# hkust-vgd/pointwise

Hardware: AMD Instinct MI355X
Metric: conv3p fwd+bwd Mpoints/s (higher is better)
Workload: dtype f32; 1 GPU; cfg2 ModelNet40-shaped: B=32 clouds/GPU x N=2048, pointcnn2_acsd conv3p stack 3->9 s1, 9->9 s2, 9->9 s3, 9->9 s4 (+SELU), forward+backward, a different batch every step, next batch's neighbour search enqueued on a side stream under the current backward; global_batch=32, points_per_cloud=2048, parallelism=dp1, backward_kernel_choice=hint from Conv3pStack.tune() at set-up: short lists

## Files before the change

pointwise_amd/csrc/conv3p_search_fused.hpp:

```cpp
#pragma once

#include "conv3p_device.hpp"

namespace conv3p {

constexpr int kFR = 16;
constexpr int kFK = 96;
constexpr int kFEntries = 116;
constexpr int kFHeader = 3 * kFEntries;
constexpr int kFTableU64 = kFHeader + 4;
constexpr int kFMaxExt = 8;
#ifndef CONV3P_DEV_FUSED_ABLATE
#define CONV3P_DEV_FUSED_ABLATE 0
#endif
constexpr int kFStream = 192;
constexpr int kFMaxE = 12;

__device__ __forceinline__ int floor_i32(float x)
{
    int r;
    asm("v_cvt_flr_i32_f32_e32 %0, %1" : "=v"(r) : "v"(x));
    return r;
}
__device__ __forceinline__ bool finite3(float x, float y, float z)
{
    return (x - x) + (y - y) + (z - z) == 0.0f;
}

__host__ __device__ constexpr int fused_window(int es) { return (kFR >> es) >= 1 ? (kFR >> es) + 1 : 2; }
static_assert(kFEntries >= kFK + fused_window(0) + 1 && kFEntries % 2 == 0, "window entries per axis");

template <typename T>
__global__ __launch_bounds__(256) void tile_tables_kernel(const PointRec<T> *__restrict__ pts, int ntiles, float inv16,
                                                          unsigned long long *__restrict__ tables,
                                                          const uint32_t *__restrict__ version,
                                                          uint32_t *__restrict__ tab_version,
                                                          uint32_t *__restrict__ tab_ticket,
                                                          uint32_t *__restrict__ tab_inv,
                                                          int force)
{
    __shared__ __attribute__((aligned(16))) unsigned long long tab[kWavesPerBlock][kFTableU64];
    const int wave = threadIdx.x >> 6, lane = threadIdx.x & 63;
    const int tile = blockIdx.x * kWavesPerBlock + wave;
    const int b = blockIdx.y;
    if (tile >= ntiles) return;
    if (!force && tab_version[b] == version[b] && tab_inv[b] == __builtin_bit_cast(uint32_t, inv16)) return;
    const size_t t = (size_t)b * ntiles + tile;
    const PointRec<T> r = pts[t * kTile + lane];
    const float v[3] = {(float)r.x, (float)r.y, (float)r.z};
    const bool valid = r.idx >= 0 && finite3(v[0], v[1], v[2]);
    float tmin[3], ext = 0.0f;
#pragma unroll
    for (int a = 0; a < 3; ++a) {
        tmin[a] = wave_min(valid ? v[a] : __builtin_huge_valf());
        const float tmax = wave_max(valid ? v[a] : -__builtin_huge_valf());
        ext = fmaxf(ext, (tmax - tmin[a]) * inv16);
    }
    const uint64_t allv = __ballot(valid);
    int e = 0;
    if (allv == 0) {
        tmin[0] = tmin[1] = tmin[2] = 0.0f;
    } else if (!(ext < 1.0e30f)) {
        e = kFMaxE + 1;
    } else {
        while (e <= kFMaxE && floor_i32(ext) >> e > kFK - 1) ++e;
    }
    const int es = e > 31 ? 31 : e;
    const int ws = fused_window(es);
    int beta[3];
#pragma unroll
    for (int a = 0; a < 3; ++a) {
        int b16 = floor_i32((v[a] - tmin[a]) * inv16) >> es;
        b16 = b16 < 0 ? 0 : (b16 > kFK - 1 ? kFK - 1 : b16);
        beta[a] = b16;
    }
    unsigned long long *mytab = tab[wave];
    {
        uint4 *z = reinterpret_cast<uint4 *>(mytab);
        for (int i = lane; i < kFTableU64 / 2; i += 64) z[i] = make_uint4(0, 0, 0, 0);
    }
    __builtin_amdgcn_wave_barrier();
    if (valid) {
        const unsigned long long bit = 1ull << lane;
        for (int i = 1; i <= ws; ++i) {
#pragma unroll
            for (int a = 0; a < 3; ++a) atomicOr(&mytab[a * kFEntries + beta[a] + i], bit);
        }
    }
    __builtin_amdgcn_wave_barrier();
    if (lane == 0) {
        mytab[kFHeader + 0] = (uint64_t)__builtin_bit_cast(uint32_t, tmin[0]) | ((uint64_t)__builtin_bit_cast(uint32_t, tmin[1]) << 32);
        mytab[kFHeader + 1] = (uint64_t)__builtin_bit_cast(uint32_t, tmin[2]) | ((uint64_t)(uint32_t)e << 32);
        mytab[kFHeader + 2] = allv;
        mytab[kFHeader + 3] = 0;
    }
    __builtin_amdgcn_wave_barrier();
    __builtin_amdgcn_s_waitcnt(0xc07f);
    const uint4 *src = reinterpret_cast<const uint4 *>(mytab);
    uint4 *dst = reinterpret_cast<uint4 *>(tables + t * kFTableU64);
    for (int i = lane; i < kFTableU64 / 2; i += 64) dst[i] = src[i];
    if (!force && lane == 0) {
        const uint32_t done = atomicAdd(&tab_ticket[b], 1u);
        if (done + 1u == (uint32_t)ntiles) {
            tab_inv[b] = __builtin_bit_cast(uint32_t, inv16);
            tab_version[b] = version[b];
            tab_ticket[b] = 0;
        }
    }
}

template <typename T> struct FusedJob {
    Stencil<T> st;
    CacheCtl cc;
    int32_t *count, *tcount;
    PairEntry *pairs;
    uint2 *segs, *qsegs;
    uint32_t *qbm, *qbm_hi;
    float clo[3][kFMaxExt];
};
constexpr int kFusedMaxJobs = 8;
template <typename T> struct FusedJobs {
    FusedJob<T> job[kFusedMaxJobs];
};

struct FusedLds {
    size_t tapmap, cnt, cen, bmk, nqw, misc, red, tab, masks, stream, total;
};
__host__ __device__ inline size_t f_a16(size_t x) { return (x + 15) & ~(size_t)15; }
__host__ __device__ inline FusedLds fused_lds(int ntap, int maxfull, int elem, int M)
{
    FusedLds L;
    size_t off = 0;
    L.tapmap = off; off += f_a16((size_t)3 * maxfull * 2);
    L.cnt = off; off += f_a16((size_t)ntap * kCntStride * 4);
    L.cen = off; off += (size_t)64 * 12 * elem;
    L.bmk = off; off += (ntap > 64 ? 256 : ntap > 32 ? 128 : 64) * 4;
    L.nqw = off; off += (size_t)kWavesPerBlock * 64 * 4;
    L.misc = off; off += 16;
    L.red = off; off += 6 * 8;
    off = f_a16(off);
    L.tab = off; off += (size_t)kWavesPerBlock * kFTableU64 * 8;
    L.masks = off; off += (size_t)kWavesPerBlock * M * 64 * 8;
    L.stream = off; off += (size_t)kWavesPerBlock * 2 * kFStream * 4;
    L.total = off;
    return L;
}

template <typename T>
__device__ __forceinline__ uint64_t tiles_meeting(const T *__restrict__ cloud_box, int ntiles, int base, const T *ulo, const T *uhi)
{
    const int t = base + (threadIdx.x & 63);
    bool ov = false;
    if (t < ntiles) {
        const T *bb = cloud_box + (size_t)t * 6;
        const T b0 = bb[0], b1 = bb[1], b2 = bb[2], b3 = bb[3], b4 = bb[4], b5 = bb[5];
        ov = !((b3 < ulo[0]) | (b0 > uhi[0]) | (b4 < ulo[1]) | (b1 > uhi[1]) | (b5 < ulo[2]) | (b2 > uhi[2]));
    }
    return __ballot(ov);
}

template <typename T>
__device__ __forceinline__ uint64_t fused_mask(const FusedJob<T> &job, const unsigned long long *tab, const float *gs, const float *fz,
                                               bool qvalid, int e)
{
    uint64_t H = ~0ull;
#pragma unroll
    for (int a = 0; a < 3; ++a) {
        uint64_t A = 0;
        const unsigned long long *ta = tab + a * kFEntries;
        for (int k = 0; k < job.st.ext[a]; ++k) {
            const float x = gs[a] + job.clo[a][k];
            int j = floor_i32(x) >> e, jh = floor_i32(x + fz[a]) >> e;
            j = j < 0 ? 0 : (j > kFEntries - 1 ? kFEntries - 1 : j);
            jh = jh < 0 ? 0 : (jh > kFEntries - 1 ? kFEntries - 1 : jh);
            A |= ta[j];
            if (__any(qvalid && jh != j)) A |= ta[jh];
        }
        H &= A;
    }
    return H;
}

template <typename T> struct TapFast {
    static constexpr bool enabled = false;
};
template <> struct TapFast<float> {
    static constexpr bool enabled = true;
};
__device__ __forceinline__ float min3_t(float a, float b, float c) { return fminf(fminf(a, b), c); }
__device__ __forceinline__ double min3_t(double a, double b, double c) { return fmin(fmin(a, b), c); }
__device__ __forceinline__ int clamp_tap(int t, int full)
{
    t = t > full - 1 ? full - 1 : t;
    return t < 0 ? 0 : t;
}

template <typename T> struct __attribute__((aligned(16))) CenRec {
    T lo[3], hi[3], p[3];
    T pad[3];
};

template <typename T>
__device__ __forceinline__ void fused_resolve(const Stencil<T> &st, T rvoxel, const int16_t *tapmap, uint32_t *cnt, uint32_t *bmk,
                                              const CenRec<T> *cen, uint32_t ql, const PointRec<T> &v, bool on, bool want_bwd,
                                              bool want_bm, uint32_t &fwd, uint32_t &bwd)
{
    const CenRec<T> c = cen[ql];
    const T d[3] = {v.x - c.lo[0], v.y - c.lo[1], v.z - c.lo[2]};
    const T dm = min3_t(d[0], d[1], d[2]);
    const T em = min3_t(c.hi[0] - v.x, c.hi[1] - v.y, c.hi[2] - v.z);
    const bool in = on && dm >= (T)0 && em >= (T)0;
    const T vv[3] = {v.x, v.y, v.z};
    fwd = kNoTap;
    bwd = kNoTap;
    bool exact = in;
    if (TapFast<T>::enabled) {
        int t[3];
        bool near = false;
#pragma unroll
        for (int a = 0; a < 3; ++a) {
            const float q = (float)d[a] * (float)rvoxel;
            const float mag = fmaxf(fabsf((float)c.p[a]), fabsf((float)vv[a]));
            near |= fabsf(q - __builtin_rintf(q)) <= __builtin_fmaf(mag, 5.0e-7f * (float)rvoxel, 1.0e-6f * (float)st.full[a]);
            t[a] = (int)q;
        }
        exact = in && near;
        if (in && !near) {
            const int tx = tapmap[clamp_tap(t[0], st.full[0])];
            const int ty = tapmap[st.maxfull + clamp_tap(t[1], st.full[1])];
            const int tz = tapmap[2 * st.maxfull + clamp_tap(t[2], st.full[2])];
            if ((tx | ty | tz) >= 0) {
                fwd = (uint32_t)((tz * st.ext[1] + ty) * st.ext[0] + tx);
                bwd = (uint32_t)st.ntap - 1u - fwd;
            }
        }
    }
    if (exact) {
        const int tx = tapmap[clamp_tap((int)(d[0] / st.voxel), st.full[0])];
        const int ty = tapmap[st.maxfull + clamp_tap((int)(d[1] / st.voxel), st.full[1])];
        const int tz = tapmap[2 * st.maxfull + clamp_tap((int)(d[2] / st.voxel), st.full[2])];
        if ((tx | ty | tz) >= 0) {
            fwd = (uint32_t)((tz * st.ext[1] + ty) * st.ext[0] + tx);
            if (want_bwd) {
                const T lx = (T)((double)v.x - st.half[0]), ly = (T)((double)v.y - st.half[1]), lz = (T)((double)v.z - st.half[2]);
                const int bx = tapmap[clamp_tap((int)((c.p[0] - lx) / st.voxel), st.full[0])];
                const int by = tapmap[st.maxfull + clamp_tap((int)((c.p[1] - ly) / st.voxel), st.full[1])];
                const int bz = tapmap[2 * st.maxfull + clamp_tap((int)((c.p[2] - lz) / st.voxel), st.full[2])];
                if ((bx | by | bz) >= 0) bwd = (uint32_t)((bz * st.ext[1] + by) * st.ext[0] + bx);
            }
        }
    }
    if (fwd != kNoTap) {
        atomicAdd(&cnt[fwd * kCntStride + ql], 1u);
        if (want_bm && bwd != kNoTap) atomicOr(&bmk[ql + ((bwd >> 5) << 6)], 1u << (bwd & 31u));
    }
}

typedef int int4_a4 __attribute__((ext_vector_type(4), aligned(4)));

constexpr uint32_t kFHitsOf32Neighbours = 40;
template <typename T> __device__ __forceinline__ bool fused_compacts(const Stencil<T> &st, uint32_t tile_hits)
{
    return !(CONV3P_DEV_FUSED_ABLATE & 16) && tile_hits > kFHitsOf32Neighbours * 64u;
}

template <typename T, bool EXT3>
__global__ __launch_bounds__(256) void search_fused_kernel(const PointRec<T> *__restrict__ pts, const T *__restrict__ boxes,
                                                           const unsigned long long *__restrict__ tables, int N, int ntiles,
                                                           int ngroups, BlockMap bm, FusedJobs<T> jobs, int M, float inv16)
{
    extern __shared__ __attribute__((aligned(16))) char smem[];
    const int wave = threadIdx.x >> 6, lane = threadIdx.x & 63;
    int b, qt;
    if (!block_to_cloud(bm, b, qt)) return;
    const FusedJob<T> &job = jobs.job[blockIdx.y];
    const bool have_pairs = job.pairs != nullptr;
    if (have_pairs && slot_valid(job.cc, b)) return;
    const Stencil<T> &st = job.st;

    const FusedLds L = fused_lds(st.ntap, st.maxfull, (int)sizeof(T), M);
    int16_t *tapmap = reinterpret_cast<int16_t *>(smem + L.tapmap);
    uint32_t *cnt = reinterpret_cast<uint32_t *>(smem + L.cnt);
    CenRec<T> *cen = reinterpret_cast<CenRec<T> *>(smem + L.cen);
    uint32_t *bmk = reinterpret_cast<uint32_t *>(smem + L.bmk);
    uint32_t *nqw = reinterpret_cast<uint32_t *>(smem + L.nqw);
    uint32_t *misc = reinterpret_cast<uint32_t *>(smem + L.misc);
    T *red = reinterpret_cast<T *>(smem + L.red);
    unsigned long long *tab = reinterpret_cast<unsigned long long *>(smem + L.tab) + (size_t)wave * kFTableU64;
    unsigned long long *masks = reinterpret_cast<unsigned long long *>(smem + L.masks) + (size_t)wave * M * 64;

    const PointRec<T> *cloud_pts = pts + (size_t)b * ntiles * kTile;
    const T *cloud_box = boxes + (size_t)b * ntiles * 6;
    const unsigned long long *cloud_tab = tables + (size_t)b * ntiles * kFTableU64;
    const PointRec<T> me = cloud_pts[(size_t)qt * kTile + lane];
    const float pf[3] = {(float)me.x, (float)me.y, (float)me.z};
    const bool qvalid = me.idx >= 0 && finite3(pf[0], pf[1], pf[2]);
    const bool want_bm = job.qbm != nullptr && (st.ntap <= 32 || (st.ntap <= 128 && job.qbm_hi != nullptr));

    build_tapmap(tapmap, st.full, st.step, st.maxfull);
    for (int e = threadIdx.x; e < st.ntap * kCntStride; e += blockDim.x) cnt[e] = 0;
    if (wave == 0) {
        CenRec<T> r;
        const T p[3] = {me.x, me.y, me.z};
#pragma unroll
        for (int a = 0; a < 3; ++a) {
            r.lo[a] = (T)((double)p[a] - st.half[a]);
            r.hi[a] = (T)((double)p[a] + st.half[a]);
            r.p[a] = p[a];
            r.pad[a] = (T)0;
        }
        cen[lane] = r;
        bmk[lane] = 0;
        if (st.ntap > 32) bmk[64 + lane] = 0;
        if (st.ntap > 64) bmk[128 + lane] = bmk[192 + lane] = 0;
    } else {
        const int a = wave - 1;
        const T pa = a == 0 ? me.x : (a == 1 ? me.y : me.z);
        const T mn = wave_min(qvalid ? pa : Limits<T>::inf()), mx = wave_max(qvalid ? pa : -Limits<T>::inf());
        if (lane == 0) {
            red[a] = mn;
            red[3 + a] = mx;
        }
    }
    const float q0[3] = {1.0e-3f + 4.0e-6f * (fabsf(pf[0]) * inv16), 1.0e-3f + 4.0e-6f * (fabsf(pf[1]) * inv16),
                         1.0e-3f + 4.0e-6f * (fabsf(pf[2]) * inv16)};
    __syncthreads();
    T ulo[3], uhi[3];
#pragma unroll
    for (int a = 0; a < 3; ++a) {
        ulo[a] = (T)((double)red[a] - st.half[a]);
        uhi[a] = (T)((double)red[3 + a] + st.half[a]);
    }
    const int S16[3] = {kFR * st.step[0], kFR * st.step[1], kFR * st.step[2]};

    auto for_my_tiles = [&](auto &&visit) {
        for (int base = 0; base < ntiles; base += 64) {
            uint64_t todo = tiles_meeting(cloud_box, ntiles, base, ulo, uhi) & (0x1111111111111111ull << wave);
            while (todo) {
                const int i = __builtin_ctzll(todo);
                todo &= todo - 1;
                visit(base + i, todo ? base + __builtin_ctzll(todo) : -1);
            }
        }
    };
    uint4 pf0 = make_uint4(0, 0, 0, 0), pf1 = pf0, pf2 = pf0;
    int pf_ct = -1;
    auto request = [&](int ct) {
        const uint4 *src = reinterpret_cast<const uint4 *>(cloud_tab + (size_t)ct * kFTableU64);
        pf0 = src[lane];
        pf1 = src[64 + lane];
        pf2 = src[128 + (lane < kFTableU64 / 2 - 128 ? lane : 0)];
        pf_ct = ct;
    };
    auto compute_mask = [&](int ct, int nxt) -> uint64_t {
        if (pf_ct != ct) request(ct);
        uint4 *dst = reinterpret_cast<uint4 *>(tab);
        __builtin_amdgcn_wave_barrier();
        dst[lane] = pf0;
        dst[64 + lane] = pf1;
        if (lane < kFTableU64 / 2 - 128) dst[128 + lane] = pf2;
        __builtin_amdgcn_wave_barrier();
        if (nxt >= 0) request(nxt);
        if (CONV3P_DEV_FUSED_ABLATE & 4) return 0ull;
        const uint64_t h0 = tab[kFHeader], h1 = tab[kFHeader + 1];
        const float tmin[3] = {__builtin_bit_cast(float, (uint32_t)h0), __builtin_bit_cast(float, (uint32_t)(h0 >> 32)),
                               __builtin_bit_cast(float, (uint32_t)h1)};
        const int e = (int)(uint32_t)(h1 >> 32);
        const int es = e > kFMaxE ? kFMaxE : e;
        const int ws = fused_window(es);
        float gs[3], fz[3], smax = 0.0f;
#pragma unroll
        for (int a = 0; a < 3; ++a) {
            const float g = (pf[a] - tmin[a]) * inv16;
            const float slack = __builtin_fmaf(4.0e-6f, fabsf(g), q0[a]);
            smax = fmaxf(smax, slack);
            gs[a] = (g - slack) + (float)(ws << es);
            fz[a] = 2.5f * slack;
        }
        const bool wide = e > kFMaxE || __any(qvalid && !(smax <= 0.2f * (float)(1 << es)));
        auto entry = [&](int i, int d) {
            const int j = (int)((uint32_t)i + (uint32_t)d) >> es;
            return j < 0 ? 0 : (j > kFEntries - 1 ? kFEntries - 1 : j);
        };
        uint64_t h;
        if (wide) {
            h = tab[kFHeader + 2];
        } else if (EXT3) {
            uint64_t A[3];
            int ih[3];
            bool far[3];
#pragma unroll
            for (int a = 0; a < 3; ++a) {
                const float x1 = gs[a] - (float)(kFR / 2);
                const int i1 = floor_i32(x1);
                ih[a] = floor_i32(x1 + fz[a]);
                far[a] = ((i1 ^ ih[a]) >> es) != 0;
                const unsigned long long *ta = tab + a * kFEntries;
                const uint64_t r0 = ta[entry(i1, -S16[a])], r1 = ta[entry(i1, 0)], r2 = ta[entry(i1, S16[a])];
                A[a] = r0 | r1 | r2;
            }
            if (__any(qvalid && (far[0] | far[1] | far[2]))) {
#pragma unroll
                for (int a = 0; a < 3; ++a) {
                    if (!__any(qvalid && far[a])) continue;
                    const unsigned long long *ta = tab + a * kFEntries;
                    const uint64_t r0 = ta[entry(ih[a], -S16[a])], r1 = ta[entry(ih[a], 0)], r2 = ta[entry(ih[a], S16[a])];
                    A[a] |= r0 | r1 | r2;
                }
            }
            h = A[0] & A[1] & A[2];
        } else {
            h = fused_mask(job, tab, gs, fz, qvalid, es);
        }
        return qvalid ? h : 0ull;
    };

    {
        uint32_t mine = 0;
        int ord = 0;
        for_my_tiles([&](int ct, int nxt) {
            const uint64_t m = compute_mask(ct, nxt);
            mine += (uint32_t)__popcll(m);
            if (ord < M) masks[(size_t)ord * 64 + lane] = m;
            ++ord;
        });
        nqw[wave * 64 + lane] = mine;
    }
    __syncthreads();

    if (wave == 0) {
        const uint32_t n0 = nqw[lane], n1 = nqw[64 + lane], n2 = nqw[128 + lane], n3 = nqw[192 + lane];
        const uint32_t nq = n0 + n1 + n2 + n3;
        int Ltot;
        const uint32_t offq = (uint32_t)wave_excl_scan((int)nq, Ltot);
        const uint32_t cap = job.cc.pairs_per_cloud;
        uint32_t base = 0, ok = 0;
        if (!have_pairs) {
            if (lane == 0) misc[0] = misc[1] = misc[2] = 0;
        } else {
        if (lane == 0) {
            base = Ltot ? atomicAdd(&job.cc.cursor[b], (uint32_t)Ltot) : 0u;
            ok = (base <= cap && (uint32_t)Ltot <= cap - base) ? 1u : 0u;
            if (!ok) atomicSub(&job.cc.cursor[b], (uint32_t)Ltot);
            base += (uint32_t)b * cap;
            job.segs[((size_t)b * ntiles + qt) * ngroups] = ok ? make_uint2(base, (uint32_t)Ltot) : make_uint2(0u, kSegOverflow);
            for (int g = 1; g < ngroups; ++g) job.segs[((size_t)b * ntiles + qt) * ngroups + g] = make_uint2(0u, 0u);
            misc[0] = base;
            misc[1] = ok;
            misc[2] = (uint32_t)Ltot;
        }
        base = __shfl(base, 0);
        ok = __shfl(ok, 0);
        if (!ok || !fused_compacts(st, (uint32_t)Ltot))
            job.qsegs[((size_t)b * ntiles + qt) * ngroups * 64 + lane] = ok ? make_uint2(base + offq, nq) : make_uint2(0u, kSegOverflow);
        for (int g = 1; g < ngroups; ++g) job.qsegs[(((size_t)b * ntiles + qt) * ngroups + g) * 64 + lane] = make_uint2(0u, 0u);
        }
        nqw[lane] = offq;
        nqw[64 + lane] = offq + n0;
        nqw[128 + lane] = offq + n0 + n1;
        nqw[192 + lane] = offq + n0 + n1 + n2;
    }
    __syncthreads();
    const bool ok = misc[1] != 0;
    const uint32_t gbase = misc[0];
    char *pbase = reinterpret_cast<char *>(job.pairs + gbase);
    const T rvoxel = (T)1 / st.voxel;

    if (!(CONV3P_DEV_FUSED_ABLATE & 2)) {
        uint32_t *sdesc = reinterpret_cast<uint32_t *>(smem + L.stream) + wave * (2 * kFStream);
        uint32_t *sslot = sdesc + kFStream;
        uint32_t off = nqw[wave * 64 + lane] * 8u;
        int have = 0, ord = 0;
        pf_ct = -1;
        auto drain = [&](int n) {
            if (CONV3P_DEV_FUSED_ABLATE & 1) return;
            constexpr int kU = 2;
            uint32_t d[kU], so[kU];
            PointRec<T> v[kU];
#pragma unroll
            for (int u = 0; u < kU; ++u) {
                const int i = u * 64 + lane;
                d[u] = sdesc[i < n ? i : 0];
                so[u] = sslot[i < n ? i : 0];
            }
#pragma unroll
            for (int u = 0; u < kU; ++u) v[u] = cloud_pts[(size_t)((d[u] >> 12) * kTile + (d[u] & 63u))];
#pragma unroll
            for (int u = 0; u < kU; ++u) {
                const bool on = u * 64 + lane < n;
                const uint32_t ql = (d[u] >> 6) & 63u;
                uint32_t fwd, bwd;
                fused_resolve<T>(st, rvoxel, tapmap, cnt, bmk, cen, ql, v[u], on, true, want_bm, fwd, bwd);
                if (on && ok) {
                    PairEntry pe;
                    pe.cand = (uint32_t)v[u].idx;
                    pe.code = pair_code(fwd, bwd, ql);
                    *reinterpret_cast<PairEntry *>(pbase + so[u]) = pe;
                }
            }
        };
        for_my_tiles([&](int ct, int nxt) {
            uint64_t mm = ord < M ? masks[(size_t)ord * 64 + lane] : compute_mask(ct, nxt);
            ++ord;
            const uint32_t dbase = ((uint32_t)ct << 12) | ((uint32_t)lane << 6);
            while (true) {
                const uint64_t act = __ballot(mm != 0);
                if (act == 0) break;
                if (mm != 0) {
                    const uint32_t c = (uint32_t)__builtin_ctzll(mm);
                    mm &= mm - 1;
                    const int at = have + (int)__builtin_amdgcn_mbcnt_hi((uint32_t)(act >> 32), __builtin_amdgcn_mbcnt_lo((uint32_t)act, 0));
                    sdesc[at] = dbase | c;
                    sslot[at] = off;
                    off += 8u;
                }
                have += __popcll(act);
                __builtin_amdgcn_wave_barrier();
                if (have >= 128) {
                    drain(128);
                    __builtin_amdgcn_wave_barrier();
                    const uint32_t cd = sdesc[128 + lane], cs = sslot[128 + lane];
                    __builtin_amdgcn_wave_barrier();
                    sdesc[lane] = cd;
                    sslot[lane] = cs;
                    have -= 128;
                    __builtin_amdgcn_wave_barrier();
                }
            }
        });
        if (have > 0) drain(have);
    }
    __threadfence_block();
    __syncthreads();

    if (have_pairs && ok && fused_compacts(st, misc[2])) {
        uint32_t *livec = nqw + 64;
        {
            const int c = wave * 16 + (lane & 15);
            uint32_t sacc = 0;
            for (int f = lane >> 4; f < st.ntap; f += 4) sacc += cnt[f * kCntStride + c];
            sacc += lane_xor16(sacc);
            sacc += lane_xor32(sacc);
            if (lane < 16) livec[c] = sacc;
        }
        __builtin_amdgcn_wave_barrier();
        const uint32_t r0 = nqw[wave * 16], r1 = wave == kWavesPerBlock - 1 ? misc[2] : nqw[wave * 16 + 16];
        PairEntry *tp = job.pairs + gbase;
        const uint64_t lt = lane == 0 ? 0ull : (~0ull >> (64 - lane));
        uint32_t carry = 0;
        constexpr int kCB = 4;
        PairEntry cur[kCB], nxt[kCB];
        auto request = [&](PairEntry (&dst)[kCB], uint32_t pos) {
#pragma unroll
            for (int u = 0; u < kCB; ++u) {
                const uint32_t i = pos + (uint32_t)(u * 64 + lane);
                dst[u] = tp[i < r1 ? i : r0];
            }
        };
        if (r0 < r1) request(nxt, r0);
        for (uint32_t pos = r0; pos < r1; pos += 64 * kCB) {
#pragma unroll
            for (int u = 0; u < kCB; ++u) cur[u] = nxt[u];
            if (pos + 64 * kCB < r1) request(nxt, pos + 64 * kCB);
#pragma unroll
            for (int u = 0; u < kCB; ++u) {
                const uint32_t cpos = pos + (uint32_t)(u * 64);
                if (cpos >= r1) break;
                const uint32_t i = cpos + (uint32_t)lane;
                const bool valid = i < r1;
                const uint32_t c = code_q(cur[u].code) & 63u;
                const bool live = valid && code_fwd(cur[u].code) != kNoTap;
                const uint32_t oc = nqw[c], lv = livec[c];
                const uint64_t Lm = __ballot(live);
                const uint32_t sc = oc > cpos ? oc - cpos : 0u;
                const uint64_t before = Lm & lt & ~((1ull << (sc & 63u)) - 1ull);
                const uint32_t rank = (uint32_t)__popcll(before) + (oc < cpos ? carry : 0u);
                if (live && oc + rank != i) tp[oc + rank] = cur[u];
                if (valid && i - oc >= lv) {
                    PairEntry dead;
                    dead.cand = cur[u].cand;
                    dead.code = pair_code(kNoTap, kNoTap, c);
                    tp[i] = dead;
                }
                carry = (uint32_t)__builtin_amdgcn_readlane((int)(rank + (live ? 1u : 0u)), 63);
            }
        }
        if (lane < 16) {
            const int c = wave * 16 + lane;
            job.qsegs[((size_t)b * ntiles + qt) * ngroups * 64 + c] = make_uint2(gbase + nqw[c], livec[c]);
        }
    }

    if (!(CONV3P_DEV_FUSED_ABLATE & 8)) {
        if (job.count != nullptr && me.idx >= 0) {
            int32_t *row = job.count + ((size_t)b * N + me.idx) * st.ntap;
            const int pieces = st.ntap >> 2;
            for (int pc = wave; pc < pieces; pc += kWavesPerBlock) {
                const uint32_t *src = cnt + (size_t)(pc * 4) * kCntStride + lane;
                int4_a4 w;
                w.x = (int)src[0];
                w.y = (int)src[kCntStride];
                w.z = (int)src[2 * kCntStride];
                w.w = (int)src[3 * kCntStride];
                *reinterpret_cast<int4_a4 *>(row + pc * 4) = w;
            }
            if (wave == (pieces & 3))
                for (int f = pieces * 4; f < st.ntap; ++f) row[f] = (int32_t)cnt[f * kCntStride + lane];
        }
        if (job.tcount != nullptr) {
            int32_t *tc = job.tcount + ((size_t)b * ntiles + qt) * st.ntap * kTile;
            for (int f = wave; f < st.ntap; f += kWavesPerBlock) tc[f * kTile + lane] = (int32_t)cnt[f * kCntStride + lane];
        }
        if (want_bm && wave == 0) {
            job.qbm[((size_t)b * ntiles + qt) * 64 + lane] = bmk[lane];
            if (st.ntap > 32) job.qbm_hi[((size_t)b * ntiles + qt) * 64 + lane] = bmk[64 + lane];
            if (st.ntap > 64) {
                const size_t pstride = (size_t)(job.qbm_hi - job.qbm);
                job.qbm_hi[pstride + ((size_t)b * ntiles + qt) * 64 + lane] = bmk[128 + lane];
                job.qbm_hi[2 * pstride + ((size_t)b * ntiles + qt) * 64 + lane] = bmk[192 + lane];
            }
        }
    }
    __syncthreads();
    if (threadIdx.x == 0 && have_pairs) {
        const CacheCtl &cc = job.cc;
        const uint32_t t = atomicAdd(&cc.ticket[b], 1u);
        if (t + 1u == (uint32_t)bm.blocks_per_cloud) {
            cc.built_version[b] = cc.version[b];
            cc.built_tag[b] = cc.tag;
            cc.ticket[b] = 0;
        }
    }
}

}
```

Before: 172.6 Mpoints/s.

## Pipeline tile-table prefetch and point gathers in fused neighbour search

Restructures the fused search kernel's tile walk into a double-buffered prefetch chain. The first tile tables are requested before the tapmap and LDS setup, and the second pass's prefetch is issued before the block barrier. The cross-wave LDS reduction for the query bounding box, and its __syncthreads, is replaced by the precomputed tile box, with a per-wave fallback. The drain step is split into issue/finish so point loads for one batch overlap with resolving the previous batch. It also adds a waves_per_eu(4) occupancy hint and readfirstlane uniform values, which may raise register pressure or limit occupancy.

```diff
diff --git a/pointwise_amd/csrc/conv3p_search_fused.hpp b/pointwise_amd/csrc/conv3p_search_fused.hpp
--- a/pointwise_amd/csrc/conv3p_search_fused.hpp
+++ b/pointwise_amd/csrc/conv3p_search_fused.hpp
@@ -12,6 +12,9 @@
 constexpr int kFMaxExt = 8;
 #ifndef CONV3P_DEV_FUSED_ABLATE
 #define CONV3P_DEV_FUSED_ABLATE 0
+#endif
+#ifndef CONV3P_DEV_FUSED_CHAIN
+#define CONV3P_DEV_FUSED_CHAIN 7
 #endif
 constexpr int kFStream = 192;
 constexpr int kFMaxE = 12;
@@ -124,7 +127,7 @@
 };
 
 struct FusedLds {
-    size_t tapmap, cnt, cen, bmk, nqw, misc, red, tab, masks, stream, total;
+    size_t tapmap, cnt, cen, bmk, nqw, misc, tab, masks, stream, total;
 };
 __host__ __device__ inline size_t f_a16(size_t x) { return (x + 15) & ~(size_t)15; }
 __host__ __device__ inline FusedLds fused_lds(int ntap, int maxfull, int elem, int M)
@@ -137,13 +140,24 @@
     L.bmk = off; off += (ntap > 64 ? 256 : ntap > 32 ? 128 : 64) * 4;
     L.nqw = off; off += (size_t)kWavesPerBlock * 64 * 4;
     L.misc = off; off += 16;
-    L.red = off; off += 6 * 8;
     off = f_a16(off);
     L.tab = off; off += (size_t)kWavesPerBlock * kFTableU64 * 8;
     L.masks = off; off += (size_t)kWavesPerBlock * M * 64 * 8;
     L.stream = off; off += (size_t)kWavesPerBlock * 2 * kFStream * 4;
     L.total = off;
     return L;
+}
+
+__device__ __forceinline__ float wave_uniform(float v)
+{
+    return __builtin_bit_cast(float, __builtin_amdgcn_readfirstlane(__builtin_bit_cast(int, v)));
+}
+__device__ __forceinline__ double wave_uniform(double v)
+{
+    const uint64_t u = __builtin_bit_cast(uint64_t, v);
+    const uint32_t lo = (uint32_t)__builtin_amdgcn_readfirstlane((int)(uint32_t)u);
+    const uint32_t hi = (uint32_t)__builtin_amdgcn_readfirstlane((int)(uint32_t)(u >> 32));
+    return __builtin_bit_cast(double, (uint64_t)lo | ((uint64_t)hi << 32));
 }
 
 template <typename T>
@@ -265,12 +279,12 @@
 }
 
 template <typename T, bool EXT3>
-__global__ __launch_bounds__(256) void search_fused_kernel(const PointRec<T> *__restrict__ pts, const T *__restrict__ boxes,
+__global__ __launch_bounds__(256) __attribute__((amdgpu_waves_per_eu(4))) void search_fused_kernel(const PointRec<T> *__restrict__ pts, const T *__restrict__ boxes,
                                                            const unsigned long long *__restrict__ tables, int N, int ntiles,
                                                            int ngroups, BlockMap bm, FusedJobs<T> jobs, int M, float inv16)
 {
     extern __shared__ __attribute__((aligned(16))) char smem[];
-    const int wave = threadIdx.x >> 6, lane = threadIdx.x & 63;
+    const int wave = __builtin_amdgcn_readfirstlane((int)(threadIdx.x >> 6)), lane = threadIdx.x & 63;
     int b, qt;
     if (!block_to_cloud(bm, b, qt)) return;
     const FusedJob<T> &job = jobs.job[blockIdx.y];
@@ -285,7 +299,6 @@
     uint32_t *bmk = reinterpret_cast<uint32_t *>(smem + L.bmk);
     uint32_t *nqw = reinterpret_cast<uint32_t *>(smem + L.nqw);
     uint32_t *misc = reinterpret_cast<uint32_t *>(smem + L.misc);
-    T *red = reinterpret_cast<T *>(smem + L.red);
     unsigned long long *tab = reinterpret_cast<unsigned long long *>(smem + L.tab) + (size_t)wave * kFTableU64;
     unsigned long long *masks = reinterpret_cast<unsigned long long *>(smem + L.masks) + (size_t)wave * M * 64;
 
@@ -297,6 +310,104 @@
     const bool qvalid = me.idx >= 0 && finite3(pf[0], pf[1], pf[2]);
     const bool want_bm = job.qbm != nullptr && (st.ntap <= 32 || (st.ntap <= 128 && job.qbm_hi != nullptr));
 
+    const T *qbox = cloud_box + (size_t)qt * 6;
+    T ulo[3], uhi[3];
+#pragma unroll
+    for (int a = 0; a < 3; ++a) {
+        ulo[a] = qbox[a];
+        uhi[a] = qbox[3 + a];
+    }
+    if (__ballot(me.idx >= 0 && !qvalid) != 0) {
+        const T p[3] = {me.x, me.y, me.z};
+#pragma unroll
+        for (int a = 0; a < 3; ++a) {
+            ulo[a] = wave_min(qvalid ? p[a] : Limits<T>::inf());
+            uhi[a] = wave_max(qvalid ? p[a] : -Limits<T>::inf());
+        }
+    }
+#pragma unroll
+    for (int a = 0; a < 3; ++a) {
+        ulo[a] = wave_uniform((T)((double)ulo[a] - st.half[a]));
+        uhi[a] = wave_uniform((T)((double)uhi[a] + st.half[a]));
+    }
+
+    const uint64_t mine_of64 = 0x1111111111111111ull << wave;
+    const uint64_t todo0 = tiles_meeting(cloud_box, ntiles, 0, ulo, uhi) & mine_of64;
+    struct TileIter {
+        int base;
+        uint64_t todo;
+    };
+    auto next_tile = [&](TileIter &it) -> int {
+        while (it.todo == 0) {
+            if (it.base + 64 >= ntiles) return -1;
+            it.base += 64;
+            it.todo = tiles_meeting(cloud_box, ntiles, it.base, ulo, uhi) & mine_of64;
+        }
+        const int i = __builtin_ctzll(it.todo);
+        it.todo &= it.todo - 1;
+        return it.base + i;
+    };
+    struct TabRegs {
+        uint4 r0, r1, r2;
+    };
+    TabRegs ta = {make_uint4(0, 0, 0, 0), make_uint4(0, 0, 0, 0), make_uint4(0, 0, 0, 0)}, tb = ta;
+    auto request = [&](TabRegs &r, int ct) {
+        const uint4 *src = reinterpret_cast<const uint4 *>(cloud_tab + (size_t)ct * kFTableU64);
+        r.r0 = src[lane];
+        r.r1 = src[64 + lane];
+        r.r2 = src[128 + (lane < kFTableU64 / 2 - 128 ? lane : 0)];
+    };
+    auto stage = [&](const TabRegs &r) {
+        uint4 *dst = reinterpret_cast<uint4 *>(tab);
+        __builtin_amdgcn_wave_barrier();
+        dst[lane] = r.r0;
+        dst[64 + lane] = r.r1;
+        if (lane < kFTableU64 / 2 - 128) dst[128 + lane] = r.r2;
+        __builtin_amdgcn_wave_barrier();
+    };
+    struct Walk {
+        TileIter rq, vs;
+    };
+    auto walk_begin = [&](int skip) {
+        Walk w = {{0, todo0}, {0, todo0}};
+        for (int k = 0; k < skip; ++k)
+            if (next_tile(w.rq) < 0) break;
+        int r = next_tile(w.rq);
+        if (r >= 0) request(ta, r);
+        if (CONV3P_DEV_FUSED_CHAIN & 2) {
+            r = next_tile(w.rq);
+            if (r >= 0) request(tb, r);
+        }
+        return w;
+    };
+    auto walk_tiles = [&](Walk &w, int skip, auto &&visit) {
+        int ord = 0, ct;
+        for (; ord < skip; ++ord) {
+            if ((ct = next_tile(w.vs)) < 0) return;
+            visit(ct, ord, false);
+        }
+        while (true) {
+            if ((ct = next_tile(w.vs)) < 0) return;
+            stage(ta);
+            {
+                const int r = next_tile(w.rq);
+                if (r >= 0) request(ta, r);
+            }
+            visit(ct, ord++, true);
+            if (CONV3P_DEV_FUSED_CHAIN & 2) {
+                if ((ct = next_tile(w.vs)) < 0) return;
+                stage(tb);
+                {
+                    const int r = next_tile(w.rq);
+                    if (r >= 0) request(tb, r);
+                }
+                visit(ct, ord++, true);
+            }
+        }
+    };
+    Walk walk1;
+    if (CONV3P_DEV_FUSED_CHAIN & 1) walk1 = walk_begin(0);
+
     build_tapmap(tapmap, st.full, st.step, st.maxfull);
     for (int e = threadIdx.x; e < st.ntap * kCntStride; e += blockDim.x) cnt[e] = 0;
     if (wave == 0) {
@@ -313,54 +424,11 @@
         bmk[lane] = 0;
         if (st.ntap > 32) bmk[64 + lane] = 0;
         if (st.ntap > 64) bmk[128 + lane] = bmk[192 + lane] = 0;
-    } else {
-        const int a = wave - 1;
-        const T pa = a == 0 ? me.x : (a == 1 ? me.y : me.z);
-        const T mn = wave_min(qvalid ? pa : Limits<T>::inf()), mx = wave_max(qvalid ? pa : -Limits<T>::inf());
-        if (lane == 0) {
-            red[a] = mn;
-            red[3 + a] = mx;
-        }
-    }
-    const float q0[3] = {1.0e-3f + 4.0e-6f * (fabsf(pf[0]) * inv16), 1.0e-3f + 4.0e-6f * (fabsf(pf[1]) * inv16),
-                         1.0e-3f + 4.0e-6f * (fabsf(pf[2]) * inv16)};
-    __syncthreads();
-    T ulo[3], uhi[3];
-#pragma unroll
-    for (int a = 0; a < 3; ++a) {
-        ulo[a] = (T)((double)red[a] - st.half[a]);
-        uhi[a] = (T)((double)red[3 + a] + st.half[a]);
     }
     const int S16[3] = {kFR * st.step[0], kFR * st.step[1], kFR * st.step[2]};
-
-    auto for_my_tiles = [&](auto &&visit) {
-        for (int base = 0; base < ntiles; base += 64) {
-            uint64_t todo = tiles_meeting(cloud_box, ntiles, base, ulo, uhi) & (0x1111111111111111ull << wave);
-            while (todo) {
-                const int i = __builtin_ctzll(todo);
-                todo &= todo - 1;
-                visit(base + i, todo ? base + __builtin_ctzll(todo) : -1);
-            }
-        }
-    };
-    uint4 pf0 = make_uint4(0, 0, 0, 0), pf1 = pf0, pf2 = pf0;
-    int pf_ct = -1;
-    auto request = [&](int ct) {
-        const uint4 *src = reinterpret_cast<const uint4 *>(cloud_tab + (size_t)ct * kFTableU64);
-        pf0 = src[lane];
-        pf1 = src[64 + lane];
-        pf2 = src[128 + (lane < kFTableU64 / 2 - 128 ? lane : 0)];
-        pf_ct = ct;
-    };
-    auto compute_mask = [&](int ct, int nxt) -> uint64_t {
-        if (pf_ct != ct) request(ct);
-        uint4 *dst = reinterpret_cast<uint4 *>(tab);
-        __builtin_amdgcn_wave_barrier();
-        dst[lane] = pf0;
-        dst[64 + lane] = pf1;
-        if (lane < kFTableU64 / 2 - 128) dst[128 + lane] = pf2;
-        __builtin_amdgcn_wave_barrier();
-        if (nxt >= 0) request(nxt);
+    if (!(CONV3P_DEV_FUSED_CHAIN & 1)) walk1 = walk_begin(0);
+
+    auto mask_staged = [&]() -> uint64_t {
         if (CONV3P_DEV_FUSED_ABLATE & 4) return 0ull;
         const uint64_t h0 = tab[kFHeader], h1 = tab[kFHeader + 1];
         const float tmin[3] = {__builtin_bit_cast(float, (uint32_t)h0), __builtin_bit_cast(float, (uint32_t)(h0 >> 32)),
@@ -372,7 +440,8 @@
 #pragma unroll
         for (int a = 0; a < 3; ++a) {
             const float g = (pf[a] - tmin[a]) * inv16;
-            const float slack = __builtin_fmaf(4.0e-6f, fabsf(g), q0[a]);
+            const float q0 = 1.0e-3f + 4.0e-6f * (fabsf(pf[a]) * inv16);
+            const float slack = __builtin_fmaf(4.0e-6f, fabsf(g), q0);
             smax = fmaxf(smax, slack);
             gs[a] = (g - slack) + (float)(ws << es);
             fz[a] = 2.5f * slack;
@@ -417,15 +486,15 @@
 
     {
         uint32_t mine = 0;
-        int ord = 0;
-        for_my_tiles([&](int ct, int nxt) {
-            const uint64_t m = compute_mask(ct, nxt);
+        walk_tiles(walk1, 0, [&](int, int ord, bool) {
+            const uint64_t m = mask_staged();
             mine += (uint32_t)__popcll(m);
             if (ord < M) masks[(size_t)ord * 64 + lane] = m;
-            ++ord;
         });
         nqw[wave * 64 + lane] = mine;
     }
+    Walk walk2 = {{0, 0}, {0, 0}};
+    if (!(CONV3P_DEV_FUSED_ABLATE & 2) && (CONV3P_DEV_FUSED_CHAIN & 1)) walk2 = walk_begin(M);
     __syncthreads();
 
     if (wave == 0) {
@@ -470,38 +539,44 @@
         uint32_t *sdesc = reinterpret_cast<uint32_t *>(smem + L.stream) + wave * (2 * kFStream);
         uint32_t *sslot = sdesc + kFStream;
         uint32_t off = nqw[wave * 64 + lane] * 8u;
-        int have = 0, ord = 0;
-        pf_ct = -1;
-        auto drain = [&](int n) {
+        int have = 0;
+        if (!(CONV3P_DEV_FUSED_CHAIN & 1)) walk2 = walk_begin(M);
+        constexpr int kU = 2;
+        uint32_t pd[kU] = {}, pso[kU] = {};
+        PointRec<T> pv[kU] = {};
+        int pn = 0;
+        auto issue = [&](int n) {
             if (CONV3P_DEV_FUSED_ABLATE & 1) return;
-            constexpr int kU = 2;
-            uint32_t d[kU], so[kU];
-            PointRec<T> v[kU];
 #pragma unroll
             for (int u = 0; u < kU; ++u) {
                 const int i = u * 64 + lane;
-                d[u] = sdesc[i < n ? i : 0];
-                so[u] = sslot[i < n ? i : 0];
-            }
-#pragma unroll
-            for (int u = 0; u < kU; ++u) v[u] = cloud_pts[(size_t)((d[u] >> 12) * kTile + (d[u] & 63u))];
+                pd[u] = sdesc[i < n ? i : 0];
+                pso[u] = sslot[i < n ? i : 0];
+            }
+#pragma unroll
+            for (int u = 0; u < kU; ++u) pv[u] = cloud_pts[(size_t)((pd[u] >> 12) * kTile + (pd[u] & 63u))];
+            pn = n;
+        };
+        auto finish = [&]() {
+            if (pn == 0) return;
 #pragma unroll
             for (int u = 0; u < kU; ++u) {
-                const bool on = u * 64 + lane < n;
-                const uint32_t ql = (d[u] >> 6) & 63u;
+                const bool on = u * 64 + lane < pn;
+                const uint32_t ql = (pd[u] >> 6) & 63u;
                 uint32_t fwd, bwd;
-                fused_resolve<T>(st, rvoxel, tapmap, cnt, bmk, cen, ql, v[u], on, true, want_bm, fwd, bwd);
+                fused_resolve<T>(st, rvoxel, tapmap, cnt, bmk, cen, ql, pv[u], on, true, want_bm, fwd, bwd);
                 if (on && ok) {
                     PairEntry pe;
-                    pe.cand = (uint32_t)v[u].idx;
+                    pe.cand = (uint32_t)pv[u].idx;
                     pe.code = pair_code(fwd, bwd, ql);
-                    *reinterpret_cast<PairEntry *>(pbase + so[u]) = pe;
+                    *reinterpret_cast<PairEntry *>(pbase + pso[u]) = pe;
                 }
-            }
+                __builtin_amdgcn_sched_barrier(0);
+            }
+            pn = 0;
         };
-        for_my_tiles([&](int ct, int nxt) {
-            uint64_t mm = ord < M ? masks[(size_t)ord * 64 + lane] : compute_mask(ct, nxt);
-            ++ord;
+        walk_tiles(walk2, M, [&](int ct, int ord, bool staged) {
+            uint64_t mm = staged ? mask_staged() : masks[(size_t)ord * 64 + lane];
             const uint32_t dbase = ((uint32_t)ct << 12) | ((uint32_t)lane << 6);
             while (true) {
                 const uint64_t act = __ballot(mm != 0);
@@ -517,7 +592,13 @@
                 have += __popcll(act);
                 __builtin_amdgcn_wave_barrier();
                 if (have >= 128) {
-                    drain(128);
+                    if (CONV3P_DEV_FUSED_CHAIN & 4) {
+                        finish();
+                        issue(128);
+                    } else {
+                        issue(128);
+                        finish();
+                    }
                     __builtin_amdgcn_wave_barrier();
                     const uint32_t cd = sdesc[128 + lane], cs = sslot[128 + lane];
                     __builtin_amdgcn_wave_barrier();
@@ -528,7 +609,11 @@
                 }
             }
         });
-        if (have > 0) drain(have);
+#pragma clang loop unroll(disable)
+        for (int last = 0; last < 2; ++last) {
+            finish();
+            if (last == 0 && have > 0) issue(have);
+        }
     }
     __threadfence_block();
     __syncthreads();
```

Result: slower. 169.1 Mpoints/s (-2.0%).
